# aleflabo/COSKAD

Hardware: AMD Instinct MI355X
Metric: pose_clips_per_sec_fwd_bwd (higher is better)
Workload: dtype f32; 1 GPU; euclidean_encoder_dynamicCenter train step (fwd+mse-to-centre+L2 reg+bwd+Adam), synthetic clips B=4096/GPU T=12 V=17 C=2, channels 2-32-16-32-64, latent 16; clips_per_gpu=4096, global_batch=4096, head=euclidean, parallelism=dp1, hip_graph=False

## Files before the change

coskad_amd/csrc/fused_bwd.hip:

```cpp
#include "fused_ops.h"
#include "layer_launch.h"

namespace coskad {
namespace fb {

using namespace ff;

constexpr int PR_A = 0, PR_XA = 12, PR_XB = 13, PR_C = 14, PR_T = 15, PR_N = 32, EROW = PR_N * 256;
constexpr int RE = 32;
__global__ __launch_bounds__(1024) void k_reduce_fused(const float* __restrict__ partials, int P, float* __restrict__ dA,
                                                       float* __restrict__ dT, const float* __restrict__ dap, int ndap,
                                                       float* __restrict__ dslope, int accumulate, const float* __restrict__ brows,
                                                       int bP, int bE, double* __restrict__ bout) {
  __shared__ double sh[1024];
  constexpr int NB = EROW / RE;
  const int col = threadIdx.x % RE;
  if ((int)blockIdx.x > NB) {
    const int e = ((int)blockIdx.x - NB - 1) * RE + col;
    const double t = column_sum_f64<RE>(brows, bP, (size_t)bE, e, e < bE, sh);
    if ((int)threadIdx.x < RE && e < bE) bout[e] = t;
    return;
  }
  if ((int)blockIdx.x == NB) {
    if (!dap) return;
    double s = 0.0;
    for (int i = threadIdx.x; i < ndap; i += 1024) s += (double)dap[i];
    sh[threadIdx.x] = s;
    __syncthreads();
    for (int w = 512; w > 0; w >>= 1) {
      if ((int)threadIdx.x < w) sh[threadIdx.x] += sh[threadIdx.x + w];
      __syncthreads();
    }
    if (threadIdx.x == 0) dslope[0] = accumulate ? dslope[0] + (float)sh[0] : (float)sh[0];
    return;
  }
  const int e = blockIdx.x * RE + col;
  const double t = column_sum_f64<RE>(partials, P, (size_t)EROW, e, true, sh);
  if ((int)threadIdx.x < RE) {
    const int rec = e >> 8, l = (e >> 2) & 63, r = e & 3, j = l & 15, q = l >> 4;
    float* out = nullptr;
    if (rec < PR_XA) out = dA + rec * V * V + (4 * q + r) * V + j;
    else if (rec == PR_XA) { if (4 * q + r < T) out = dA + (4 * q + r) * V * V + 16 * V + j; }
    else if (rec == PR_XB) { if (4 * q + r < T) out = dA + (4 * q + r) * V * V + j * V + 16; }
    else if (rec == PR_C) { if (r == 0 && q == 0 && j < T) out = dA + j * V * V + 16 * V + 16; }
    else if (4 * q + r < T && j < T) out = dT + (rec - PR_T) * T * T + (4 * q + r) * T + j;
    if (out) *out = accumulate ? *out + (float)t : (float)t;
  }
}

constexpr int bpc_occ(int CT, int NS) { return CT == 1 && NS == 0 ? 3 : 2; }
constexpr bool bpc_tlds(int CT, int OT, int NS) { return bpc_occ(CT, NS) == 2 && OT < 4; }
constexpr int TF_F = V * 3 * 64, AS_F = T * 5 * 64, ET_F = 256;
constexpr int bpc_lds_floats(int CT, int OT, int NS) {
  return WAVE_LDS_W + 4 * 256 + (bpc_tlds(CT, OT, NS) ? TF_F + AS_F + ET_F + CT * CT * 256 + 2 * 16 * CT : 0);
}
#ifndef FBB_BDBL
#define FBB_BDBL 0
#endif
#ifndef FBB_SKIP
#define FBB_SKIP 0
#endif

template <int CT, int OT, int NS, int CB>
__global__ __launch_bounds__(256, bpc_occ(CT, NS)) void k_layer_bwd_bpc(const float* __restrict__ in, const float* __restrict__ Zg,
                                                               const float* __restrict__ dU, const float* __restrict__ coef,
                                                               const float* __restrict__ btab, const float* __restrict__ in_slope,
                                                               float* __restrict__ dIn, float* __restrict__ partials,
                                                               float* __restrict__ dap, int B, const float* __restrict__ below_z,
                                                               const float* __restrict__ below_x, const float* __restrict__ below_slope,
                                                               float* __restrict__ below_stats) {
  constexpr int Ci = 16 * CT, Co = 16 * OT, CiP = Ci, NG = OT + CT;
  constexpr int KT0 = (Co + Ci) * CiP, DX0 = KT0 + CiP, KR0 = DX0 + (Co + Ci) * CiP;
  constexpr int MAXF = CT == 2 ? 6 : 3;
  extern __shared__ __attribute__((aligned(16))) float lds[];
  float* r1 = lds;
  float* r2 = lds + 32 * LD;
  float* zs = lds + WAVE_LDS_W + 256 * (threadIdx.x >> 6);
  constexpr bool TLDS = bpc_tlds(CT, OT, NS);
  float* tf = lds + WAVE_LDS_W + 4 * 256;
  float* as = tf + TF_F;
  float* et = as + AS_F;
  float* krl = et + ET_F;
  float* kql = krl + CT * CT * 256;
  const int tid = threadIdx.x, lane = tid & 63;
  const int wave = __builtin_amdgcn_readfirstlane(tid >> 6);
  auto geo = [&]() {
    int l = lane;
    asm volatile("" : "+v"(l));
    return Lane{l & 15, l >> 4};
  };
  Lane L = geo();
  const float a_in = in_slope[0];
  const int l16 = lane * 16;
  const BufRes tabres = make_res(btab, BTAB_F4 * 16u);
  const BufRes cres = make_res(coef, (KR0 + CiP) * 4u);
  auto clip_res = [&](const float* base, int c, int rows) {
    const bool in_range = c < B;
#ifdef COSKAD_HOT
    return make_res(base + (size_t)(in_range ? (c & 63) : 0) * rows * TV, in_range ? rows * TV * 4u : 0u);
#else
    return make_res(base + (size_t)(in_range ? c : 0) * rows * TV, in_range ? rows * TV * 4u : 0u);
#endif
  };
  const int ct = CT == 2 ? (wave & 1) : 0;
  const int f0 = CT == 2 ? 6 * (wave >> 1) : 3 * wave;
  const bool owns16 = CT == 2 ? (wave >> 1) == 1 : wave == 3;
  constexpr int Q4 = 4 * (TV / 4);
  const bool stg = tid < Q4;
  const int srow = tid / (TV / 4), scol = 4 * (tid - srow * (TV / 4));
  const int svoff = stg ? tid * 16 : 0x7ffffff0;
  auto qload = [&](const BufRes& res, int row0, int q) { return buf_load4(res, svoff, (row0 + 4 * q) * (TV / 4) * 16); };
  auto qstore = [&](int q, float4 v, bool act, float slope, int stride) {
    if (act) { v.x = prelu(v.x, slope); v.y = prelu(v.y, slope); v.z = prelu(v.z, slope); v.w = prelu(v.w, slope); }
    *reinterpret_cast<float2*>(r2 + (stg ? (4 * q + srow) * stride + scol : 15 * stride + PADCOL)) = float2{v.x, v.y};
    *reinterpret_cast<float2*>(r2 + (stg ? (4 * q + srow) * stride + scol + 2 : 15 * stride + PADCOL)) = float2{v.z, v.w};
  };
  constexpr int N4 = Ci * (TV / 4), XL = (N4 + 255) / 256;
  float4 xs[XL];
  auto xload = [&](float4 (&dst)[XL], const BufRes& r) {
#pragma unroll
    for (int i = 0; i < XL; ++i) dst[i] = buf_load4(r, (tid + 256 * i) < N4 ? (tid + 256 * i) * 16 : 0x7ffffff0, 0);
  };
  f32x4 dAacc[MAXF], exA = {0.f, 0.f, 0.f, 0.f}, exB = {0.f, 0.f, 0.f, 0.f};
  constexpr int MAXJ = (V + 3) / 4;
  f32x4 dTacc[MAXJ];
  float corner = 0.f, da = 0.f;
#pragma unroll
  for (int t = 0; t < MAXF; ++t) dAacc[t] = f32x4{0.f, 0.f, 0.f, 0.f};
#pragma unroll
  for (int k = 0; k < MAXJ; ++k) dTacc[k] = f32x4{0.f, 0.f, 0.f, 0.f};
  constexpr int NGB = NS == 2 ? 2 * CB : 1;
  f32x4 nsb[NGB][CT];
  float nss[CT];
#pragma unroll
  for (int g = 0; g < NGB; ++g)
#pragma unroll
    for (int c = 0; c < CT; ++c) nsb[g][c] = f32x4{0.f, 0.f, 0.f, 0.f};
#pragma unroll
  for (int c = 0; c < CT; ++c) nss[c] = 0.f;
  const bool bpre = NS != 0 && below_slope != nullptr;
  const float a_b = bpre ? below_slope[0] : 0.f;

  auto temporal_rr = [&](int base4, auto from_lds) {
    const Lane Lt = geo();
    auto trec = [&](int v) {
      if constexpr (decltype(from_lds)::value) {
        const float* p = tf + v * 192 + 16 * Lt.q + Lt.j;
        return float4{p[0], p[64], p[128], 0.f};
      } else {
        return buf_load4(tabres, l16, (base4 + v * 64) * 16);
      }
    };
    TOp cur[CT], nxt[CT];
    f32x4 dprev[CT];
    int vprev = -1;
#pragma unroll
    for (int rt = 0; rt < CT; ++rt) cur[rt] = temporal_read<16>(r1, rt, wave, Lt);
    float4 rec = trec(wave);
    for (int v = wave; v < V; v += 4) {
      const int vn = v + 4 < V ? v + 4 : v;
      const float4 recn = trec(vn);
#pragma unroll
      for (int rt = 0; rt < CT; ++rt) nxt[rt] = temporal_read<16>(r1, rt, vn, Lt);
      f32x4 d[CT];
#pragma unroll
      for (int rt = 0; rt < CT; ++rt) d[rt] = temporal_mm(cur[rt], rec);
      if (vprev >= 0) {
#pragma unroll
        for (int rt = 0; rt < CT; ++rt) temporal_store<16>(r1, rt, vprev, dprev[rt], Lt);
      }
#pragma unroll
      for (int rt = 0; rt < CT; ++rt) { dprev[rt] = d[rt]; cur[rt] = nxt[rt]; }
      vprev = v;
      rec = recn;
    }
#pragma unroll
    for (int rt = 0; rt < CT; ++rt) temporal_store<16>(r1, rt, vprev, dprev[rt], Lt);
  };
  auto spatial_rr = [&]() {
    const Lane Ls = geo();
    auto spat_rec = [&](int t) {
      if constexpr (TLDS) {
        const float* p = as + t * 320 + 16 * Ls.q + Ls.j;
        const float* e = et + t * 20 + Ls.q;
        return SpatRec{float4{p[0], p[64], p[128], p[192]}, float4{p[256], e[0], e[4], e[8]}, float4{e[12], e[16], 0.f, 0.f}};
      } else {
        return load_spat(tabres, 0, t, l16);
      }
    };
    SpatRec srec = spat_rec(wave);
    SOp op[CT];
#pragma unroll
    for (int rt = 0; rt < CT; ++rt) op[rt] = spatial_read<16>(r1, rt, wave, Ls);
#pragma unroll
    for (int k = 0; k < T / 4; ++k) {
      const int t = wave + 4 * k, tn = k + 1 < T / 4 ? t + 4 : t;
      const SpatRec nrec = spat_rec(tn);
      SOp opn[CT];
#pragma unroll
      for (int rt = 0; rt < CT; ++rt) opn[rt] = spatial_read<16>(r1, rt, tn, Ls);
#pragma unroll
      for (int rt = 0; rt < CT; ++rt) {
        const f32x4 d = spatial_mm(op[rt], srec);
        spatial_extra<16>(r1, rt, t, op[rt], srec, Ls);
        tile_store(r1, 16 * rt, t * V + Ls.j, true, d, Ls);
      }
      srec = nrec;
#pragma unroll
      for (int rt = 0; rt < CT; ++rt) op[rt] = opn[rt];
    }
  };

  auto stage_params = [&]() {
    for (int e = tid; e < V * 64; e += 256) {
      const float4 r = buf_load4(tabres, e * 16, 0);
      float* p = tf + (e >> 6) * 192 + (e & 63);
      p[0] = r.x; p[64] = r.y; p[128] = r.z;
    }
    for (int e = tid; e < T * 64; e += 256) {
      const int t = e >> 6, l = e & 63, o = (TEMP_F4 + t * 3 * 64 + l) * 16;
      const float4 c0 = buf_load4(tabres, o, 0), c1 = buf_load4(tabres, o, 1024), c2 = buf_load4(tabres, o, 2048);
      float* p = as + t * 320 + l;
      p[0] = c0.x; p[64] = c0.y; p[128] = c0.z; p[192] = c0.w; p[256] = c1.x;
      if ((l & 15) == 0) {
        float* q = et + t * 20 + (l >> 4);
        q[0] = c1.y; q[4] = c1.z; q[8] = c1.w; q[12] = c2.x; q[16] = c2.y;
      }
    }
    for (int e = tid; e < CT * CT * 256; e += 256) {
      const int l = e & 63, c = (e >> 6) % CT, hs = (e >> 6) / CT;
      krl[e] = buf_load1(cres, ((DX0 / CiP + Co + 4 * hs + (l >> 4)) * CiP + 16 * c + (l & 15)) * 4, 0);
    }
    if (tid < 2 * Ci) kql[tid] = buf_load1(cres, ((tid < Ci ? KT0 : KR0 - Ci) + tid) * 4, 0);
  };
  int clip = blockIdx.x;
  float4 gq[4];
  {
    xload(xs, clip_res(in, clip, Ci));
    const BufRes du0 = clip_res(dU, clip, Co);
#pragma unroll
    for (int q = 0; q < 4; ++q) gq[q] = qload(du0, 0, q);
  }
  if constexpr (TLDS) stage_params();
  for (; clip < B; clip += gridDim.x) {
    const BufRes xres = clip_res(in, clip, Ci), zres = clip_res(Zg, clip, Ci), dures = clip_res(dU, clip, Co);
    const BufRes ores = clip_res(dIn, clip, Ci);
    auto kload = [&](int g, int q, const BufRes& res2) { return g < OT ? qload(dures, 16 * g, q) : qload(res2, 16 * (g - OT), q); };
    __syncthreads();
#pragma unroll
    for (int i = 0; i < XL; ++i) {
      const int e4 = tid + 256 * i;
      float4 v = xs[i];
      v.x = prelu(v.x, a_in); v.y = prelu(v.y, a_in); v.z = prelu(v.z, a_in); v.w = prelu(v.w, a_in);
      const int row = e4 / (TV / 4), col = 4 * (e4 - row * (TV / 4));
      *reinterpret_cast<float2*>(r1 + (e4 < N4 ? row * LD + col : PADCOL)) = float2{v.x, v.y};
      *reinterpret_cast<float2*>(r1 + (e4 < N4 ? row * LD + col + 2 : PADCOL)) = float2{v.z, v.w};
    }
#pragma unroll
    for (int q = 0; q < 4; ++q) {
      qstore(q, gq[q], false, 0.f, LDW);
      gq[q] = kload(1, q, zres);
    }
    __syncthreads();
    if (!(FBB_SKIP & 1)) temporal_rr(0, std::integral_constant<bool, TLDS>{});
    L = geo();
    const int lq = (L.q * CiP + 16 * ct + L.j) * 4;
    const int jc = L.j < T ? L.j : T - 1;
    auto pos_of = [&](int k) { return k < MAXF ? (f0 + k) * V + L.j : jc * V + 16; };
    auto kpass = [&](f32x4 (&acc)[MAXF + 1], f32x4 (&acc2)[MAXF + 1], const BufRes& res2, bool act2, int c0, int c1, int c2,
                     bool with16, bool with16b) {
      constexpr bool DUAL = true;
      float wc[2][4], wc2[2][4];
      auto cload = [&](int buf, int g) {
        const int krow = g < OT ? c0 + 16 * g : c1 + 16 * (g - OT);
#pragma unroll
        for (int s = 0; s < 4; ++s) {
          wc[buf][s] = buf_load1(cres, lq, ((krow + 4 * s) * CiP) * 4);
          if (DUAL && g < OT) wc2[buf][s] = buf_load1(cres, lq, ((c2 + 16 * g + 4 * s) * CiP) * 4);
        }
      };
      cload(0, 0);
      float b[1 + FBB_BDBL][MAXF + 1];
#pragma unroll
      for (int k = 0; k <= MAXF; ++k) b[0][k] = r2[L.q * LDW + pos_of(k)];
#pragma unroll
      for (int g = 0; g < NG; ++g) {
        if (g + 1 < NG) cload((g + 1) & 1, g + 1);
#pragma unroll
        for (int s = 0; s < 4; ++s) {
          if (g + 1 < NG || s == 0) __syncthreads();
          const int sn = (s + 1) & 3;
          if (FBB_BDBL && (s + 1 < 4 || g + 1 < NG)) {
            __builtin_amdgcn_sched_barrier(0);
#pragma unroll
            for (int k = 0; k <= MAXF; ++k) b[(s + 1) & 1][k] = r2[(4 * sn + L.q) * LDW + pos_of(k)];
            __builtin_amdgcn_sched_barrier(0);
          }
          if (g + 1 < NG) {
            qstore(s, gq[s], g + 1 >= OT && act2, a_in, LDW);
            if (g + 2 < NG) gq[s] = kload(g + 2, s, res2);
          }
#pragma unroll
          for (int k = 0; k <= MAXF; ++k)
            if (k < MAXF || with16) acc[k] = mfma(wc[g & 1][s], b[FBB_BDBL ? (s & 1) : 0][k], acc[k]);
          if (DUAL && g < OT) {
#pragma unroll
            for (int k = 0; k <= MAXF; ++k)
              if (k < MAXF || with16b) acc2[k] = mfma(wc2[g & 1][s], b[FBB_BDBL ? (s & 1) : 0][k], acc2[k]);
          }
          if (!FBB_BDBL && (s + 1 < 4 || g + 1 < NG)) {
#pragma unroll
            for (int k = 0; k <= MAXF; ++k) b[0][k] = r2[(4 * sn + L.q) * LDW + pos_of(k)];
          }
        }
      }
    };
    f32x4 az[MAXF + 1];
    {
      const float4 a = TLDS ? *reinterpret_cast<const float4*>(kql + 16 * ct + 4 * L.q) : buf_load4(cres, L.q * 16, (KT0 + 16 * ct) * 4);
#pragma unroll
      for (int k = 0; k <= MAXF; ++k) az[k] = f32x4{a.x, a.y, a.z, a.w};
    }
    f32x4 xr[MAXF + 1];
    {
      const float4 kq = TLDS ? *reinterpret_cast<const float4*>(kql + Ci + 16 * ct + 4 * L.q) : buf_load4(cres, L.q * 16, (KR0 + 16 * ct) * 4);
#pragma unroll
      for (int k = 0; k <= MAXF; ++k) xr[k] = f32x4{kq.x, kq.y, kq.z, kq.w};
    }
    __syncthreads();
    if (!(FBB_SKIP & 2)) kpass(az, xr, zres, false, 0, Co, DX0 / CiP, true, owns16);
#pragma unroll
    for (int q = 0; q < 4; ++q) gq[q] = qload(xres, 0, q);
    if (owns16) {
      const f32x4 y16 = tile_load(r1, 16 * ct, jc * V + 16, L);
#pragma unroll
      for (int r = 0; r < 4; ++r) corner = fmaf(y16[r], az[MAXF][r], corner);
    }
    *reinterpret_cast<f32x4*>(zs + lane * 4) = az[MAXF];
#pragma unroll
    for (int k = 0; k < ((FBB_SKIP & 4) ? 0 : MAXF); ++k) {
      const int t = f0 + k;
      const f32x4 y = tile_load(r1, 16 * ct, t * V + L.j, L);
      const f32x4 y16 = tile_load(r1, 16 * ct, t * V + 16, L);
      const f32x4 dz16 = *reinterpret_cast<const f32x4*>(zs + (16 * L.q + t) * 4);
      float pa = 0.f, pb = 0.f;
#pragma unroll
      for (int r = 0; r < 4; ++r) {
        dAacc[k] = mfma(y[r], az[k][r], dAacc[k]);
        pa = fmaf(y16[r], az[k][r], pa);
        pb = fmaf(y[r], dz16[r], pb);
      }
      const float sel = L.j == t ? 1.f : 0.f;
      exA = mfma(sel, pa, exA);
      exB = mfma(sel, pb, exB);
    }
    __syncthreads();
#pragma unroll
    for (int k = 0; k < MAXF; ++k) tile_store(r1, 16 * ct, (f0 + k) * V + L.j, true, az[k], L);
    if (owns16) tile_store(r1, 16 * ct, jc * V + 16, L.j < T, az[MAXF], L);
    __syncthreads();
    if (!(FBB_SKIP & 8)) spatial_rr();
    __syncthreads();
    L = geo();
    {
      const int ic = L.j < T ? L.j : T - 1;
#pragma unroll
      for (int h = 0; h < ((FBB_SKIP & 16) ? 0 : CT); ++h) {
#pragma unroll
        for (int q = 0; q < 4; ++q) {
          qstore(q, gq[q], true, a_in, LDW);
          if (h + 1 < CT) gq[q] = qload(xres, 16 * (h + 1), q);
        }
        float wk[4];
#pragma unroll
        for (int s = 0; s < 4; ++s)
          wk[s] = TLDS ? krl[((4 * h + s) * CT + ct) * 64 + 16 * L.q + L.j] : buf_load1(cres, lq, ((DX0 / CiP + Co + 16 * h + 4 * s) * CiP) * 4);
        __syncthreads();
#pragma unroll
        for (int s = 0; s < 4; ++s) {
          if (!(FBB_SKIP & 2)) {
            float bx[MAXF + 1];
#pragma unroll
            for (int k = 0; k <= MAXF; ++k) bx[k] = r2[(4 * s + L.q) * LDW + pos_of(k)];
#pragma unroll
            for (int k = 0; k <= MAXF; ++k)
              if (k < MAXF || owns16) xr[k] = mfma(wk[s], bx[k], xr[k]);
          }
#pragma unroll
          for (int k = 0; k < MAXJ; ++k) {
            const int v = wave + 4 * k;
            if (v < V) {
              const float a = r2[(4 * s + L.q) * LDW + ic * V + v];
              const float bb = r1[(16 * h + 4 * s + L.q) * LD + ic * V + v];
              dTacc[k] = mfma(L.j < T ? a : 0.f, L.j < T ? bb : 0.f, dTacc[k]);
            }
          }
        }
        __syncthreads();
      }
    }
    float4 u[XL];
    {
      if (!(FBB_SKIP & 1)) temporal_rr(TEMP_F4 + SPAT_F4, std::false_type{});
      __syncthreads();
      xload(u, xres);
      L = geo();
#pragma unroll
      for (int k = 0; k < MAXF; ++k) {
        const int pos = (f0 + k) * V + L.j;
        tile_store(r1, 16 * ct, pos, true, xr[k] + tile_load(r1, 16 * ct, pos, L), L);
      }
      if (owns16) {
        const int pos = (L.j < T ? L.j : T - 1) * V + 16;
        tile_store(r1, 16 * ct, pos, L.j < T, xr[MAXF] + tile_load(r1, 16 * ct, pos, L), L);
      }
    }
    __syncthreads();
    if (!(FBB_SKIP & 32)) {
      const BufRes xn = clip_res(in, clip + gridDim.x, Ci), dun = clip_res(dU, clip + gridDim.x, Co);
      float4 pg[4];
      if constexpr (NS == 1) {
        const int fv = tid < 2 * (TV / 4) ? tid * 16 : 0x7ffffff0;
        pg[0] = buf_load4(clip_res(below_z, clip, 2), fv, 0);
        pg[1] = buf_load4(clip_res(below_x, clip, 2), fv, 0);
      }
      if constexpr (NS == 2) {
#pragma unroll
        for (int q = 0; q < 4; ++q) gq[q] = qload(clip_res(below_z, clip, 16 * CB), 0, q);
      } else {
#pragma unroll
        for (int q = 0; q < 4; ++q) gq[q] = qload(dun, 0, q);
      }
#pragma unroll
      for (int i = 0; i < XL; ++i) {
        const int e4 = tid + 256 * i;
        const int row = e4 / (TV / 4), col = 4 * (e4 - row * (TV / 4));
        float* p = r1 + (e4 < N4 ? row * LD + col : PADCOL);
        float* p2 = r1 + (e4 < N4 ? row * LD + col + 2 : PADCOL);
        const float2 g0 = *reinterpret_cast<const float2*>(p), g1 = *reinterpret_cast<const float2*>(p2);
        float g[4] = {g0.x, g0.y, g1.x, g1.y};
        if (e4 < N4) {
          const float uu[4] = {u[i].x, u[i].y, u[i].z, u[i].w};
#pragma unroll
          for (int c = 0; c < 4; ++c) {
            if (uu[c] < 0.f) da = fmaf(g[c], uu[c], da);
            g[c] = uu[c] > 0.f ? g[c] : a_in * g[c];
          }
        }
        buf_store4(ores, e4 < N4 ? e4 * 16 : 0x7ffffff0, 0, float4{g[0], g[1], g[2], g[3]});
        if constexpr (NS != 0) {
          *reinterpret_cast<float2*>(p) = float2{g[0], g[1]};
          *reinterpret_cast<float2*>(p2) = float2{g[2], g[3]};
        }
      }
      xload(xs, xn);
      if constexpr (NS == 1) {
        {
          float4 vz = pg[0], vx = pg[1];
          if (bpre) { vx.x = prelu(vx.x, a_b); vx.y = prelu(vx.y, a_b); vx.z = prelu(vx.z, a_b); vx.w = prelu(vx.w, a_b); }
          const bool fst = tid < 2 * (TV / 4);
          const int frow = tid / (TV / 4), fcol = 4 * (tid - frow * (TV / 4));
          *reinterpret_cast<float2*>(r2 + (fst ? frow * LD + fcol : 3 * LD + PADCOL)) = float2{vz.x, vz.y};
          *reinterpret_cast<float2*>(r2 + (fst ? frow * LD + fcol + 2 : 3 * LD + PADCOL)) = float2{vz.z, vz.w};
          *reinterpret_cast<float2*>(r2 + (fst ? (2 + frow) * LD + fcol : 3 * LD + PADCOL)) = float2{vx.x, vx.y};
          *reinterpret_cast<float2*>(r2 + (fst ? (2 + frow) * LD + fcol + 2 : 3 * LD + PADCOL)) = float2{vx.z, vx.w};
        }
        __syncthreads();
        L = geo();
        const float* pb = r2 + (L.j & 3) * LD + 2 * L.q;
        const float* pa = r1 + L.j * LD + 2 * L.q;
        constexpr int NM = (TV + 7) / 8;
        for (int m = wave; m < NM; m += 4) {
          float2 b = *reinterpret_cast<const float2*>(pb + 8 * m);
          const bool aok = 8 * m + 2 * L.q < TV, ok = aok && L.j < 4;
          b.x = ok ? b.x : 0.f; b.y = ok ? b.y : 0.f;
#pragma unroll
          for (int c = 0; c < CT; ++c) {
            float2 a = *reinterpret_cast<const float2*>(pa + 16 * c * LD + 8 * m);
            a.x = aok ? a.x : 0.f; a.y = aok ? a.y : 0.f;
            nsb[0][c] = mfma(a.x, b.x, nsb[0][c]);
            nsb[0][c] = mfma(a.y, b.y, nsb[0][c]);
            nss[c] += a.x + a.y;
          }
        }
#pragma unroll
        for (int q = 0; q < 4; ++q) gq[q] = qload(dun, 0, q);
      }
      if constexpr (NS == 2) {
        auto bres = [&](int g) { return g < CB ? clip_res(below_z, clip, 16 * CB) : clip_res(below_x, clip, 16 * CB); };
        auto brow = [&](int g) { return 16 * (g < CB ? g : g - CB); };
        constexpr int NM = (TV + 7) / 8;
#pragma unroll
        for (int g = 0; g < NGB; ++g) {
          __syncthreads();
#pragma unroll
          for (int q = 0; q < 4; ++q) {
            qstore(q, gq[q], g >= CB && bpre, a_b, LD);
            gq[q] = g + 1 < NGB ? qload(bres(g + 1), brow(g + 1), q) : qload(dun, 0, q);
          }
          __syncthreads();
          L = geo();
          const float* pb = r2 + L.j * LD + 2 * L.q;
          const float* pa = r1 + L.j * LD + 2 * L.q;
          for (int m = wave; m < NM; m += 4) {
            float2 b = *reinterpret_cast<const float2*>(pb + 8 * m);
            const bool ok = 8 * m + 2 * L.q < TV;
            b.x = ok ? b.x : 0.f; b.y = ok ? b.y : 0.f;
#pragma unroll
            for (int c = 0; c < CT; ++c) {
              float2 a = *reinterpret_cast<const float2*>(pa + 16 * c * LD + 8 * m);
              a.x = ok ? a.x : 0.f; a.y = ok ? a.y : 0.f;
              nsb[g][c] = mfma(a.x, b.x, nsb[g][c]);
              nsb[g][c] = mfma(a.y, b.y, nsb[g][c]);
              if (g == 0) nss[c] += a.x + a.y;
            }
          }
        }
      }
    }
  }

  __syncthreads();
  float4* row4 = reinterpret_cast<float4*>(lds);
  for (int e = tid; e < PR_N * 64; e += 256) row4[e] = float4{0.f, 0.f, 0.f, 0.f};
  float* extra = lds + PR_N * 256;
  constexpr int Cb = NS == 1 ? 2 : 16 * CB;
  constexpr int NSE = NS ? 2 * Ci * Cb + Ci : 0;
  for (int e = tid; e < 64 + NSE; e += 256) extra[e] = 0.f;
  __syncthreads();
  L = geo();
  auto add4 = [&](int rec, const f32x4& v) {
    float4 o = row4[rec * 64 + lane];
    o.x += v[0]; o.y += v[1]; o.z += v[2]; o.w += v[3];
    row4[rec * 64 + lane] = o;
  };
  da = wave_sum(da);
  for (int w = 0; w < 4; ++w) {
    if (wave == w) {
#pragma unroll
      for (int k = 0; k < MAXF; ++k) add4(PR_A + f0 + k, dAacc[k]);
      add4(PR_XA, exA);
      add4(PR_XB, exB);
      add4(PR_C, f32x4{quad_sum(corner), 0.f, 0.f, 0.f});
#pragma unroll
      for (int k = 0; k < MAXJ; ++k)
        if (wave + 4 * k < V) add4(PR_T + wave + 4 * k, dTacc[k]);
      if (lane == 0) extra[0] += da;
      if constexpr (NS == 1) {
#pragma unroll
        for (int c = 0; c < CT; ++c) {
#pragma unroll
          for (int r = 0; r < 4; ++r) {
            const int o = 16 * c + 4 * L.q + r;
            if (L.j < 4) extra[64 + (L.j < 2 ? o * 2 + L.j : 2 * Ci + o * 2 + (L.j - 2))] += nsb[0][c][r];
          }
          const float t = quad_sum(nss[c]);
          if (L.q == 0) extra[64 + 4 * Ci + 16 * c + L.j] += t;
        }
      }
      if constexpr (NS == 2) {
#pragma unroll
        for (int g = 0; g < NGB; ++g)
#pragma unroll
          for (int c = 0; c < CT; ++c)
#pragma unroll
            for (int r = 0; r < 4; ++r) {
              const int o = 16 * c + 4 * L.q + r;
              extra[64 + (g < CB ? 0 : Ci * Cb) + o * Cb + 16 * (g < CB ? g : g - CB) + L.j] += nsb[g][c][r];
            }
#pragma unroll
        for (int c = 0; c < CT; ++c) {
          const float t = quad_sum(nss[c]);
          if (L.q == 0) extra[64 + 2 * Ci * Cb + 16 * c + L.j] += t;
        }
      }
    }
    __syncthreads();
  }
  float4* prow = reinterpret_cast<float4*>(partials + (size_t)blockIdx.x * EROW);
  for (int e = tid; e < PR_N * 64; e += 256) prow[e] = row4[e];
  if (tid == 0 && dap) dap[blockIdx.x] = extra[0];
  if constexpr (NS != 0) {
    for (int e = tid; e < NSE; e += 256) below_stats[(size_t)blockIdx.x * NSE + e] = extra[64 + e];
  }
}

}

int bwd_bpc_rows(int B, int Ci, bool chain) {
  const int grid = 256 * fb::bpc_occ(Ci / 16, chain ? 1 : 0);
  return B < grid ? B : grid;
}

int launch_layer_bwd_bpc(const float* in, const float* Zg, const float* dU, const float* coef, const float* in_slope, float* dIn,
                         float* btab, float* partials, float* dap, int B, int Ci, int Co, hipStream_t st, int* rows_out,
                         const float* below_z, const float* below_x, const float* below_slope, int below_Ci, float* below_stats) {
  const int grid = bwd_bpc_rows(B, Ci, below_stats != nullptr);
  *rows_out = grid;
#define LAUNCH_FBB(CT, OT, NS, CB)                                                                                   \
  do {                                                                                                               \
    rc = launch_lds<fb::k_layer_bwd_bpc<CT, OT, NS, CB>>("bwd_bpc", dim3(grid), dim3(256),                          \
                                                         fb::bpc_lds_floats(CT, OT, NS) * sizeof(float), st, in, Zg, dU, coef,  \
                                                         (const float*)btab, in_slope, dIn, partials, dap, B, below_z,      \
                                                         below_x, below_slope, below_stats);                                \
  } while (0)
  int rc = COSKAD_OK;
  {
    ProbeScope probe(KID_BWD_DATA, Ci, Co, st);
    if (below_stats) {
      if (Ci == 32 && Co == 16 && below_Ci == 2) LAUNCH_FBB(2, 1, 1, 0);
      else if (Ci == 16 && Co == 32 && below_Ci == 32) LAUNCH_FBB(1, 2, 2, 2);
      else if (Ci == 32 && Co == 64 && below_Ci == 16) LAUNCH_FBB(2, 4, 2, 1);
      else return fail(COSKAD_ERR_SHAPE, "bwd_bpc: no kernel forms the reductions of a %d-channel layer below (%d -> %d)", below_Ci, Ci, Co);
    } else if (Ci == 16 && Co == 16) LAUNCH_FBB(1, 1, 0, 0);
    else if (Ci == 16 && Co == 32) LAUNCH_FBB(1, 2, 0, 0);
    else if (Ci == 16 && Co == 64) LAUNCH_FBB(1, 4, 0, 0);
    else if (Ci == 32 && Co == 16) LAUNCH_FBB(2, 1, 0, 0);
    else if (Ci == 32 && Co == 32) LAUNCH_FBB(2, 2, 0, 0);
    else if (Ci == 32 && Co == 64) LAUNCH_FBB(2, 4, 0, 0);
    else return fail(COSKAD_ERR_SHAPE, "bwd_bpc: unsupported channels (%d, %d)", Ci, Co);
  }
#undef LAUNCH_FBB
  return rc;
}

int launch_reduce_fused(const float* partials, int rows, float* dA, float* dT, const float* dap, float* dslope, int accumulate,
                        hipStream_t st, const float* brows, int bE, double* bout) {
  const int extra = brows ? 1 + ceil_div(bE, fb::RE) : (dap ? 1 : 0);
  hipLaunchKernelGGL(fb::k_reduce_fused, dim3(fb::EROW / fb::RE + extra), dim3(1024), 0, st, partials, rows, dA, dT, dap, rows,
                     dslope, accumulate, brows, rows, bE, bout);
  return check_launch("bwd_reduce_fused");
}

int layer_bwd_below_rows(int T_, int V_, int B, int Ci, int Co, int below_Ci) {
  const bool built = (Ci == 32 && Co == 16 && below_Ci == 2) || (Ci == 16 && Co == 32 && below_Ci == 32) ||
                     (Ci == 32 && Co == 64 && below_Ci == 16);
  if (!(T_ == ff::T && V_ == ff::V && built) || B <= 0) return 0;
  return bwd_bpc_rows(B, Ci, true);
}

bool layer_bwd_fused_ok(int T_, int V_, int Ci, int Co) {
  return T_ == ff::T && V_ == ff::V && (Ci == 16 || Ci == 32) && (Co == 16 || Co == 32 || Co == 64);
}

}
```

Measured before the change: 3.153 million clips/s.

## Park accumulators in LDS and software-pipeline LDS operand reads in bwd kernel

```diff
diff --git a/coskad_amd/csrc/fused_bwd.hip b/coskad_amd/csrc/fused_bwd.hip
--- a/coskad_amd/csrc/fused_bwd.hip
+++ b/coskad_amd/csrc/fused_bwd.hip
@@ -51,12 +51,15 @@
 constexpr int bpc_occ(int CT, int NS) { return CT == 1 && NS == 0 ? 3 : 2; }
 constexpr bool bpc_tlds(int CT, int OT, int NS) { return bpc_occ(CT, NS) == 2 && OT < 4; }
 constexpr int TF_F = V * 3 * 64, AS_F = T * 5 * 64, ET_F = 256;
-constexpr int bpc_lds_floats(int CT, int OT, int NS) {
-  return WAVE_LDS_W + 4 * 256 + (bpc_tlds(CT, OT, NS) ? TF_F + AS_F + ET_F + CT * CT * 256 + 2 * 16 * CT : 0);
-}
-#ifndef FBB_BDBL
-#define FBB_BDBL 0
-#endif
+constexpr int PK_DT = 1, PK_NS = 2;
+constexpr int bpc_park(int CT, int OT, int NS) { return CT == 2 && OT == 4 && NS == 2 ? PK_DT | PK_NS : 0; }
+constexpr int bpc_park_quads(int CT, int OT, int NS, int CB) {
+  return ((bpc_park(CT, OT, NS) & PK_DT) ? (V + 3) / 4 : 0) + ((bpc_park(CT, OT, NS) & PK_NS) ? (NS == 2 ? 2 * CB : 1) * CT : 0);
+}
+constexpr int bpc_lds_floats(int CT, int OT, int NS, int CB) {
+  return WAVE_LDS_W + 4 * 256 + (bpc_tlds(CT, OT, NS) ? TF_F + AS_F + ET_F + CT * CT * 256 + 2 * 16 * CT : 0) +
+         4 * 256 * bpc_park_quads(CT, OT, NS, CB);
+}
 #ifndef FBB_SKIP
 #define FBB_SKIP 0
 #endif
@@ -82,6 +85,10 @@
   float* et = as + AS_F;
   float* krl = et + ET_F;
   float* kql = krl + CT * CT * 256;
+  constexpr int PARK = bpc_park(CT, OT, NS);
+  static_assert(!(PARK && TLDS), "the parked sums' slots start where the parameter operands would");
+  static_assert(bpc_lds_floats(CT, OT, NS, CB) * 4 * bpc_occ(CT, NS) <= 160 * 1024, "LDS: the occupancy the registers allow");
+  f32x4* pk = reinterpret_cast<f32x4*>(lds + WAVE_LDS_W + 4 * 256) + (threadIdx.x >> 6) * bpc_park_quads(CT, OT, NS, CB) * 64 + (threadIdx.x & 63);
   const int tid = threadIdx.x, lane = tid & 63;
   const int wave = __builtin_amdgcn_readfirstlane(tid >> 6);
   auto geo = [&]() {
@@ -138,6 +145,37 @@
     for (int c = 0; c < CT; ++c) nsb[g][c] = f32x4{0.f, 0.f, 0.f, 0.f};
 #pragma unroll
   for (int c = 0; c < CT; ++c) nss[c] = 0.f;
+  auto park_dt = [&]() {
+    if constexpr ((PARK & PK_DT) != 0) {
+#pragma unroll
+      for (int k = 0; k < MAXJ; ++k) pk[64 * k] = dTacc[k];
+    }
+  };
+  auto restore_dt = [&]() {
+    if constexpr ((PARK & PK_DT) != 0) {
+#pragma unroll
+      for (int k = 0; k < MAXJ; ++k) dTacc[k] = pk[64 * k];
+    }
+  };
+  constexpr int PK_NS0 = (PARK & PK_DT) ? MAXJ : 0;
+  auto park_ns = [&]() {
+    if constexpr ((PARK & PK_NS) != 0) {
+#pragma unroll
+      for (int g = 0; g < NGB; ++g)
+#pragma unroll
+        for (int c = 0; c < CT; ++c) pk[64 * (PK_NS0 + g * CT + c)] = nsb[g][c];
+    }
+  };
+  auto restore_ns = [&]() {
+    if constexpr ((PARK & PK_NS) != 0) {
+#pragma unroll
+      for (int g = 0; g < NGB; ++g)
+#pragma unroll
+        for (int c = 0; c < CT; ++c) nsb[g][c] = pk[64 * (PK_NS0 + g * CT + c)];
+    }
+  };
+  park_dt();
+  park_ns();
   const bool bpre = NS != 0 && below_slope != nullptr;
   const float a_b = bpre ? below_slope[0] : 0.f;
 
@@ -280,7 +318,7 @@
         }
       };
       cload(0, 0);
-      float b[1 + FBB_BDBL][MAXF + 1];
+      float b[2][MAXF + 1];
 #pragma unroll
       for (int k = 0; k <= MAXF; ++k) b[0][k] = r2[L.q * LDW + pos_of(k)];
 #pragma unroll
@@ -290,7 +328,7 @@
         for (int s = 0; s < 4; ++s) {
           if (g + 1 < NG || s == 0) __syncthreads();
           const int sn = (s + 1) & 3;
-          if (FBB_BDBL && (s + 1 < 4 || g + 1 < NG)) {
+          if (s + 1 < 4 || g + 1 < NG) {
             __builtin_amdgcn_sched_barrier(0);
 #pragma unroll
             for (int k = 0; k <= MAXF; ++k) b[(s + 1) & 1][k] = r2[(4 * sn + L.q) * LDW + pos_of(k)];
@@ -302,15 +340,11 @@
           }
 #pragma unroll
           for (int k = 0; k <= MAXF; ++k)
-            if (k < MAXF || with16) acc[k] = mfma(wc[g & 1][s], b[FBB_BDBL ? (s & 1) : 0][k], acc[k]);
+            if (k < MAXF || with16) acc[k] = mfma(wc[g & 1][s], b[s & 1][k], acc[k]);
           if (DUAL && g < OT) {
 #pragma unroll
             for (int k = 0; k <= MAXF; ++k)
-              if (k < MAXF || with16b) acc2[k] = mfma(wc2[g & 1][s], b[FBB_BDBL ? (s & 1) : 0][k], acc2[k]);
-          }
-          if (!FBB_BDBL && (s + 1 < 4 || g + 1 < NG)) {
-#pragma unroll
-            for (int k = 0; k <= MAXF; ++k) b[0][k] = r2[(4 * sn + L.q) * LDW + pos_of(k)];
+              if (k < MAXF || with16b) acc2[k] = mfma(wc2[g & 1][s], b[s & 1][k], acc2[k]);
           }
         }
       }
@@ -363,7 +397,26 @@
     __syncthreads();
     L = geo();
     {
-      const int ic = L.j < T ? L.j : T - 1;
+      const bool tj = L.j < T;
+      const int ic = tj ? L.j : T - 1;
+      struct DtOps { float bx[MAXF + 1], a[MAXJ], bb[MAXJ]; };
+      auto dt_reads = [&](DtOps& o, int h, int s) {
+        const float* w = r2 + (4 * s + L.q) * LDW;
+        const float* y = r1 + (16 * h + 4 * s + L.q) * LD + ic * V;
+        if (!(FBB_SKIP & 2)) {
+#pragma unroll
+          for (int k = 0; k <= MAXF; ++k) o.bx[k] = w[pos_of(k)];
+        }
+#pragma unroll
+        for (int k = 0; k < MAXJ; ++k) {
+          const int v = k + 1 < MAXJ || wave == 0 ? wave + 4 * k : V - 1;
+          o.a[k] = w[ic * V + v];
+          o.bb[k] = y[v];
+        }
+      };
+      constexpr int DTS = bpc_occ(CT, NS) == 2 ? 2 : 1;
+      DtOps dto[DTS];
+      restore_dt();
 #pragma unroll
       for (int h = 0; h < ((FBB_SKIP & 16) ? 0 : CT); ++h) {
 #pragma unroll
@@ -376,28 +429,34 @@
         for (int s = 0; s < 4; ++s)
           wk[s] = TLDS ? krl[((4 * h + s) * CT + ct) * 64 + 16 * L.q + L.j] : buf_load1(cres, lq, ((DX0 / CiP + Co + 16 * h + 4 * s) * CiP) * 4);
         __syncthreads();
+        dt_reads(dto[0], h, 0);
 #pragma unroll
         for (int s = 0; s < 4; ++s) {
+          DtOps& o = dto[s % DTS];
+#pragma unroll
+          for (int k = 0; k < MAXJ; ++k) {
+            o.a[k] = tj ? o.a[k] : 0.f;
+            o.bb[k] = tj ? o.bb[k] : 0.f;
+          }
+          __builtin_amdgcn_sched_barrier(0);
+          if (DTS == 2 && s + 1 < 4) dt_reads(dto[(s + 1) % DTS], h, s + 1);
+          __builtin_amdgcn_sched_barrier(0);
           if (!(FBB_SKIP & 2)) {
-            float bx[MAXF + 1];
-#pragma unroll
-            for (int k = 0; k <= MAXF; ++k) bx[k] = r2[(4 * s + L.q) * LDW + pos_of(k)];
 #pragma unroll
             for (int k = 0; k <= MAXF; ++k)
-              if (k < MAXF || owns16) xr[k] = mfma(wk[s], bx[k], xr[k]);
-          }
-#pragma unroll
-          for (int k = 0; k < MAXJ; ++k) {
-            const int v = wave + 4 * k;
-            if (v < V) {
-              const float a = r2[(4 * s + L.q) * LDW + ic * V + v];
-              const float bb = r1[(16 * h + 4 * s + L.q) * LD + ic * V + v];
-              dTacc[k] = mfma(L.j < T ? a : 0.f, L.j < T ? bb : 0.f, dTacc[k]);
-            }
+              if (k < MAXF || owns16) xr[k] = mfma(wk[s], o.bx[k], xr[k]);
+          }
+#pragma unroll
+          for (int k = 0; k < MAXJ; ++k)
+            if (k + 1 < MAXJ || wave == 0) dTacc[k] = mfma(o.a[k], o.bb[k], dTacc[k]);
+          if (DTS == 1 && s + 1 < 4) {
+            __builtin_amdgcn_sched_barrier(0);
+            dt_reads(dto[0], h, s + 1);
           }
         }
         __syncthreads();
       }
+      park_dt();
     }
     float4 u[XL];
     {
@@ -454,6 +513,50 @@
         }
       }
       xload(xs, xn);
+      auto chain_products = [&](const float* pa, const float* pb, f32x4 (&acc)[CT], bool rowsum, bool bok) {
+        constexpr int NM = (TV + 7) / 8;
+        auto land = [&](int m, float2& b, float2 (&a)[CT]) {
+          const bool aok = 8 * m + 2 * L.q < TV, ok = aok && bok;
+          b.x = ok ? b.x : 0.f; b.y = ok ? b.y : 0.f;
+#pragma unroll
+          for (int c = 0; c < CT; ++c) { a[c].x = aok ? a[c].x : 0.f; a[c].y = aok ? a[c].y : 0.f; }
+        };
+        auto reads = [&](int m, float2& b, float2 (&a)[CT]) {
+          b = *reinterpret_cast<const float2*>(pb + 8 * m);
+#pragma unroll
+          for (int c = 0; c < CT; ++c) a[c] = *reinterpret_cast<const float2*>(pa + 16 * c * LD + 8 * m);
+        };
+        float2 b, a[CT], bn, an[CT];
+        reads(wave, b, a);
+        land(wave, b, a);
+        for (int m = wave; m < NM; m += 4) {
+          const int mn = m + 4 < NM ? m + 4 : m;
+          if constexpr (CT == 2) {
+            __builtin_amdgcn_sched_barrier(0);
+            reads(mn, bn, an);
+            __builtin_amdgcn_sched_barrier(0);
+            acc[0] = mfma(a[0].x, b.x, acc[0]);
+            acc[CT - 1] = mfma(a[CT - 1].x, b.x, acc[CT - 1]);
+            acc[0] = mfma(a[0].y, b.y, acc[0]);
+            acc[CT - 1] = mfma(a[CT - 1].y, b.y, acc[CT - 1]);
+          } else {
+            acc[0] = mfma(a[0].x, b.x, acc[0]);
+            __builtin_amdgcn_sched_barrier(0);
+            reads(mn, bn, an);
+            __builtin_amdgcn_sched_barrier(0);
+            acc[0] = mfma(a[0].y, b.y, acc[0]);
+          }
+          if (rowsum) {
+#pragma unroll
+            for (int c = 0; c < CT; ++c) nss[c] += a[c].x + a[c].y;
+          }
+          __builtin_amdgcn_sched_barrier(0);
+          land(mn, bn, an);
+          b = bn;
+#pragma unroll
+          for (int c = 0; c < CT; ++c) a[c] = an[c];
+        }
+      };
       if constexpr (NS == 1) {
         {
           float4 vz = pg[0], vx = pg[1];
@@ -469,27 +572,14 @@
         L = geo();
         const float* pb = r2 + (L.j & 3) * LD + 2 * L.q;
         const float* pa = r1 + L.j * LD + 2 * L.q;
-        constexpr int NM = (TV + 7) / 8;
-        for (int m = wave; m < NM; m += 4) {
-          float2 b = *reinterpret_cast<const float2*>(pb + 8 * m);
-          const bool aok = 8 * m + 2 * L.q < TV, ok = aok && L.j < 4;
-          b.x = ok ? b.x : 0.f; b.y = ok ? b.y : 0.f;
-#pragma unroll
-          for (int c = 0; c < CT; ++c) {
-            float2 a = *reinterpret_cast<const float2*>(pa + 16 * c * LD + 8 * m);
-            a.x = aok ? a.x : 0.f; a.y = aok ? a.y : 0.f;
-            nsb[0][c] = mfma(a.x, b.x, nsb[0][c]);
-            nsb[0][c] = mfma(a.y, b.y, nsb[0][c]);
-            nss[c] += a.x + a.y;
-          }
-        }
+        chain_products(pa, pb, nsb[0], true, L.j < 4);
 #pragma unroll
         for (int q = 0; q < 4; ++q) gq[q] = qload(dun, 0, q);
       }
       if constexpr (NS == 2) {
         auto bres = [&](int g) { return g < CB ? clip_res(below_z, clip, 16 * CB) : clip_res(below_x, clip, 16 * CB); };
         auto brow = [&](int g) { return 16 * (g < CB ? g : g - CB); };
-        constexpr int NM = (TV + 7) / 8;
+        restore_ns();
 #pragma unroll
         for (int g = 0; g < NGB; ++g) {
           __syncthreads();
@@ -502,24 +592,15 @@
           L = geo();
           const float* pb = r2 + L.j * LD + 2 * L.q;
           const float* pa = r1 + L.j * LD + 2 * L.q;
-          for (int m = wave; m < NM; m += 4) {
-            float2 b = *reinterpret_cast<const float2*>(pb + 8 * m);
-            const bool ok = 8 * m + 2 * L.q < TV;
-            b.x = ok ? b.x : 0.f; b.y = ok ? b.y : 0.f;
-#pragma unroll
-            for (int c = 0; c < CT; ++c) {
-              float2 a = *reinterpret_cast<const float2*>(pa + 16 * c * LD + 8 * m);
-              a.x = ok ? a.x : 0.f; a.y = ok ? a.y : 0.f;
-              nsb[g][c] = mfma(a.x, b.x, nsb[g][c]);
-              nsb[g][c] = mfma(a.y, b.y, nsb[g][c]);
-              if (g == 0) nss[c] += a.x + a.y;
-            }
-          }
-        }
+          chain_products(pa, pb, nsb[g], g == 0, true);
+        }
+        park_ns();
       }
     }
   }
 
+  restore_dt();
+  restore_ns();
   __syncthreads();
   float4* row4 = reinterpret_cast<float4*>(lds);
   for (int e = tid; e < PR_N * 64; e += 256) row4[e] = float4{0.f, 0.f, 0.f, 0.f};
@@ -600,7 +681,7 @@
 #define LAUNCH_FBB(CT, OT, NS, CB)                                                                                   \
   do {                                                                                                               \
     rc = launch_lds<fb::k_layer_bwd_bpc<CT, OT, NS, CB>>("bwd_bpc", dim3(grid), dim3(256),                          \
-                                                         fb::bpc_lds_floats(CT, OT, NS) * sizeof(float), st, in, Zg, dU, coef,  \
+                                                         fb::bpc_lds_floats(CT, OT, NS, CB) * sizeof(float), st, in, Zg, dU, coef,  \
                                                          (const float*)btab, in_slope, dIn, partials, dap, B, below_z,      \
                                                          below_x, below_slope, below_stats);                                \
   } while (0)
```

Result: faster. 3.189 million clips/s (median of 6 runs) (+1.1%).
